# Wil-Lee/NN_BVH

Hardware: AMD Instinct MI355X
Metric: Mray/s (closest-hit + any-hit) (higher is better)
Workload: dtype f32; 1 GPU; crown, 1000x1400: one wavefront pass of 8 spp per step (8 spp per GPU-film) — primary, bounce-1 and bounce-2 closest-hit, shadow any-hit towards the light quads (batches pre-generated, hence independent: ONE launch; the dependent form is dependent_step), rays in --ray-order tile (a caller-side order the reference's integrator does not form: ray_order_probe), RecordShadowRayResult + RGBFilm::AddSam; sample_sets=4, geometry=procedural stand-in for crown (3548192 tris; data/crown.npz absent), tree=sah, triangles=3548192, nodes=7032259, rays_primary=11200000, rays_bounce=7410327, rays_bounce2=4392209, parallelism=tile-sharded x1, BVH replicated, film all-gather after the pass

## Files before the change

### nn_bvh_amd/csrc/bvh_trace.hip

```cpp
#include <hip/hip_runtime.h>
#include <stdint.h>

#include "bvh_trace.h"
#include "anim_math.h"
#include "spawn_math.h"
#include "stream_access.h"
#include "trace_math.h"

namespace nnbvh {

constexpr int kDone = (int)0x80000000;
constexpr int kReturn = (int)0x80000001;
constexpr int kEnter = (int)0x80000002;

#ifndef NNBVH_MINW_CLOSEST
#define NNBVH_MINW_CLOSEST 6
#endif
#ifndef NNBVH_MINW_ANY
#define NNBVH_MINW_ANY 6
#endif
#ifndef NNBVH_LEAN_EXTRA_WAVES
#define NNBVH_LEAN_EXTRA_WAVES 2
#endif
#ifndef NNBVH_MINW_ALPHA
#define NNBVH_MINW_ALPHA 5
#endif
#ifndef NNBVH_MINW_ALPHA_PATCH
#define NNBVH_MINW_ALPHA_PATCH 3
#endif
#ifndef NNBVH_ANIM_ENTER_WEIGHT
#define NNBVH_ANIM_ENTER_WEIGHT 8
#endif
template <typename T>
__device__ __forceinline__ T pick_batch(const T (&a)[kMaxFusedBatches], int b) {
    static_assert(kMaxFusedBatches == 4, "written out for four batches");
    return b == 0 ? a[0] : (b == 1 ? a[1] : (b == 2 ? a[2] : a[3]));
}

template <int MODE, int W, int INST, int PATCH, int ALPHA = 0, int SOA = 0, int HOSTC = 0>
__global__ __launch_bounds__(kBlockThreads, (INST ? 1 : (ALPHA ? (ALPHA == 2 ? NNBVH_MINW_ALPHA_PATCH : NNBVH_MINW_ALPHA) : ((MODE == 0 || MODE == 3) ? NNBVH_MINW_CLOSEST : NNBVH_MINW_ANY) + (PATCH ? 0 : NNBVH_LEAN_EXTRA_WAVES))))
void trace_kernel(TraceParams p) {
    static_assert(PATCH || !INST, "two-level scenes need the ray direction");
    static_assert(PATCH || !ALPHA, "the alpha test hashes the ray direction");
    static_assert(!HOSTC || (PATCH && (MODE == 0 || MODE == 2 || (MODE == 3 && !ALPHA && W == 8)) && !SOA),
                  "candidate mode: general instances of modes 0 / 2 / 3");
    __shared__ float s_stack[kBlockThreads / 64][W][2][64];
    constexpr bool kLean = !PATCH && !INST;
    constexpr int kColdRi = 0, kColdD = 1, kColdHit = kLean ? 0 : (PATCH ? 4 : 1),
                  kColdHost = kColdHit + ((MODE == 0 || MODE == 3) ? 4 : 0);
    constexpr int kColdBase = kColdHost + (kLean ? 0 : 1);
    constexpr int kSaveO = kColdBase, kSaveInv = kColdBase + 3, kSaveShear = kColdBase + 6,
                  kSaveKz = kColdBase + 9, kSaveTmax = kColdBase + 10, kSaveD = kColdBase + 11,
                  kResume = kColdBase + 14, kCurInst = kColdBase + 15, kHitInst = kColdBase + 16,
                  kInnerHit = kColdBase + 17, kColdTime = kColdBase + 18, kPendSlot = kColdBase + 19;
    constexpr int kColdFields = kColdBase + (INST ? 20 : 0);
    __shared__ float s_cold[kBlockThreads / 64][kColdFields > 0 ? kColdFields : 1][64];

    const int lane = threadIdx.x & 63;
    const int wave = threadIdx.x >> 6;
    const int gtid = blockIdx.x * kBlockThreads + threadIdx.x;
    float(*stk)[2][64] = s_stack[wave];
    float(*cold)[64] = s_cold[wave];
    int riReg = -1;
    if (!kLean) cold[kColdRi][lane] = __int_as_float(-1);
    const long spillStride = (long)gridDim.x * kBlockThreads;

    int q = 0;
    if (p.nQueues > 1) {
        unsigned xcc;
        asm volatile("s_getreg_b32 %0, hwreg(HW_REG_XCC_ID)" : "=s"(xcc));
        q = (int)(xcc & 0xf) % p.nQueues;
    }
    int queuesTried = 0;
    int curBatch = 0;
    long nRays = p.n;
    if (p.nDev) {
        const long nd = (long)*p.nDev;
        nRays = nd < 0 ? 0 : (nd < nRays ? nd : nRays);
    }

#ifdef NNBVH_STATS
    unsigned long long st[16] = {0, 0, 0, 0, 0, 0, 0, 0, 0, 0, 0, 0, 0, 0, 0, 0};
    unsigned long long stPrev = __builtin_amdgcn_s_memtime();
    int stKind = 2;
#endif
    RayState r;
    RayMasks masks = {0ull, 0ull, 0ull, 0ull, 0ull, 0ull};
    float tMax = 0.0f;
    int visited = 0, tests = 0;
    int cur = kDone, sp = 0, base = 0;
    int floor = -1;
    bool found = false;
    bool exhausted = false;

    auto pop_entry = [&](int &ref, float &key) {
        --sp;
        ref = __float_as_int(stk[sp & (W - 1)][0][lane]);
        key = stk[sp & (W - 1)][1][lane];
        asm volatile("" : "+v"(ref), "+v"(key));
        if (sp < base) {
            const uint2 e = p.spill[(long)sp * spillStride + gtid];
            base = sp;
            ref = (int)e.x;
            key = __uint_as_float(e.y);
            asm volatile("" : "+v"(ref), "+v"(key));
        }
        if (MODE != 2) visited += 1;
    };
    auto pop_next = [&]() -> int {
        const int lowest = (INST && floor > 0) ? floor : 0;
        const int none = (INST && floor >= 0) ? kReturn : kDone;
        if (sp <= lowest) return none;
        int ref;
        float key;
        pop_entry(ref, key);
        if (key < tMax) return ref;
        while (sp > lowest) {
            pop_entry(ref, key);
            if (key < tMax) return ref;
        }
        return none;
    };

    auto enter_instance = [&](int slot, unsigned flags, float4 s0, float4 s1, float4 s2) {
        const float4 s3 = p.prims[slot + 3], s4 = p.prims[slot + 4], s5 = p.prims[slot + 5];
        const V3 dOuter = {cold[kColdD][lane], cold[kColdD + 1][lane], cold[kColdD + 2][lane]};
        cold[kSaveO][lane] = r.o.x;
        cold[kSaveO + 1][lane] = r.o.y;
        cold[kSaveO + 2][lane] = r.o.z;
        cold[kSaveInv][lane] = r.inv.x;
        cold[kSaveInv + 1][lane] = r.inv.y;
        cold[kSaveInv + 2][lane] = r.inv.z;
        cold[kSaveShear][lane] = r.sx;
        cold[kSaveShear + 1][lane] = r.sy;
        cold[kSaveShear + 2][lane] = r.sz;
        cold[kSaveKz][lane] = __int_as_float(r.kz);
        cold[kSaveTmax][lane] = tMax;
        cold[kSaveD][lane] = dOuter.x;
        cold[kSaveD + 1][lane] = dOuter.y;
        cold[kSaveD + 2][lane] = dOuter.z;
        cold[kResume][lane] = __int_as_float((flags & kPrimLast) ? kDone : ~(slot + 6));
        cold[kCurInst][lane] = __int_as_float(__float_as_int(s0.w) + 1);
        cold[kInnerHit][lane] = 0.0f;
        V3 oIn, dIn;
        float4 m0 = s2, m1 = s3, m2 = s4;
        if (INST == 2 && (flags & kPrimAnimated) && p.anim)
            anim_inverse_rows(p.anim + (long)kAnimStride * __float_as_int(s0.w), cold[kColdTime][lane], m0, m1, m2);
        apply_inverse_ray(m0, m1, m2, r.o, dOuter, tMax, oIn, dIn);
        r.o = oIn;
        cold[kColdD][lane] = dIn.x;
        cold[kColdD + 1][lane] = dIn.y;
        cold[kColdD + 2][lane] = dIn.z;
        r.inv = {1.0f / dIn.x, 1.0f / dIn.y, 1.0f / dIn.z};
        ray_shear(r, dIn);
        floor = sp;
        if (MODE != 2) visited += 1;
        float tEntry;
        const bool rootHit =
            slab_partial(s0.x, s0.y, s0.z, s1.x, s1.y, s1.z, r, tEntry) && (tEntry < tMax);
        cur = rootHit ? __float_as_int(s5.x) : kReturn;
    };

    auto leave_instance = [&]() {
        const bool innerHit = cold[kInnerHit][lane] != 0.0f;
        r.o = {cold[kSaveO][lane], cold[kSaveO + 1][lane], cold[kSaveO + 2][lane]};
        r.inv = {cold[kSaveInv][lane], cold[kSaveInv + 1][lane], cold[kSaveInv + 2][lane]};
        r.sx = cold[kSaveShear][lane];
        r.sy = cold[kSaveShear + 1][lane];
        r.sz = cold[kSaveShear + 2][lane];
        r.kz = __float_as_int(cold[kSaveKz][lane]);
        cold[kColdD][lane] = cold[kSaveD][lane];
        cold[kColdD + 1][lane] = cold[kSaveD + 1][lane];
        cold[kColdD + 2][lane] = cold[kSaveD + 2][lane];
        if (!innerHit) tMax = cold[kSaveTmax][lane];
        cold[kCurInst][lane] = 0.0f;
        floor = -1;
        const int resume = __float_as_int(cold[kResume][lane]);
        cur = (resume == kDone) ? pop_next() : resume;
    };

    auto prim_math = [&](const int slot, const float4 s0, const float4 s1, const float4 s2) {
        const unsigned flags = __float_as_uint(s1.w);
        if (INST && (flags & kPrimInstance)) {
            if (INST == 2 && NNBVH_ANIM_ENTER_WEIGHT > 0 && (flags & kPrimAnimated) && p.anim) {
                cold[kPendSlot][lane] = __int_as_float(slot);
                cur = kEnter;
            } else {
                enter_instance(slot, flags, s0, s1, s2);
            }
        } else if (!kLean && (flags & kPrimHost)) {
            if constexpr (HOSTC) {
                const int c = __float_as_int(cold[kColdHost][lane]);
                if (c >= 0) {
                    long ray = __float_as_int(cold[kColdRi][lane]);
                    int cap = p.hcCap;
                    int32_t *hcPrim = p.hcPrim, *hcInst = p.hcInst;
                    if constexpr (MODE == 3) {
                        const int b = (int)(ray >> kFusedIndexBits);
                        ray &= (1 << kFusedIndexBits) - 1;
                        cap = pick_batch(p.bHcCap, b);
                        hcPrim = pick_batch(p.bHcPrim, b);
                        hcInst = pick_batch(p.bHcInst, b);
                    }
                    if (c < cap) {
                        const long at = ray * cap + c;
                        hcPrim[at] = __float_as_int(s0.w);
                        hcInst[at] = INST ? __float_as_int(cold[kCurInst][lane]) : 0;
                    }
                    cold[kColdHost][lane] = __int_as_float(c < cap ? c + 1 : -1);
                }
            } else {
                cold[kColdHost][lane] = 1.0f;
            }
            cur = (flags & kPrimLast) ? pop_next() : ~(slot + 3);
        } else {
            tests += 1;
            bool hit;
            float x0, x1, x2, th;
            int next;
            if (!PATCH || !(flags & kPrimPatch)) {
                hit = triangle_test(r, tMax, (flags & kPrimDegenerate) != 0,
                                    {s0.x, s0.y, s0.z}, {s1.x, s1.y, s1.z},
                                    {s2.x, s2.y, s2.z}, x0, x1, x2, th, kLean ? &masks : nullptr);
                next = slot + ((ALPHA && (flags & kPrimSmooth)) ? 6 : 3);
                if (ALPHA && hit && (flags & kPrimAlpha)) {
                    const float a = s2.w;
                    if (a < 1) {
                        const V3 rd = {cold[kColdD][lane], cold[kColdD + 1][lane],
                                       cold[kColdD + 2][lane]};
                        const float u = (a <= 0) ? 1.f : hash_float_6f(r.o, rd);
                        if (u > a) {
                            hit = false;
                            RayState rn = r;
                            if (flags & kPrimSmooth) {
                                const float4 m0 = p.prims[slot + 3], m1 = p.prims[slot + 4], m2 = p.prims[slot + 5];
                                rn.o = alpha_retrace_origin({s0.x, s0.y, s0.z}, {s1.x, s1.y, s1.z}, {s2.x, s2.y, s2.z}, x0,
                                                            x1, x2, (flags & kPrimFlipN) != 0, rd, true, {m0.x, m0.y, m0.z},
                                                            {m1.x, m1.y, m1.z}, {m2.x, m2.y, m2.z});
                            } else {
                                rn.o = alpha_retrace_origin({s0.x, s0.y, s0.z}, {s1.x, s1.y, s1.z},
                                                            {s2.x, s2.y, s2.z}, x0, x1, x2,
                                                            (flags & kPrimFlipN) != 0, rd);
                            }
                            tests += 1;
                            float y0, y1, y2, tn;
                            if (triangle_test(rn, tMax - th, (flags & kPrimDegenerate) != 0,
                                              {s0.x, s0.y, s0.z}, {s1.x, s1.y, s1.z},
                                              {s2.x, s2.y, s2.z}, y0, y1, y2, tn))
                                cold[kColdHost][lane] = HOSTC ? __int_as_float(-2) : 1.0f;
                        }
                    }
                }
            } else {
                const float4 s3 = p.prims[slot + 3];
                x2 = 0.0f;
                const V3 rd = {cold[PATCH ? kColdD : 0][lane], cold[PATCH ? kColdD + 1 : 0][lane],
                               cold[PATCH ? kColdD + 2 : 0][lane]};
                next = slot + 4 + ((ALPHA == 2 && (flags & kPrimSmooth)) ? 4 : 0) + ((ALPHA == 2 && (flags & kPrimUV)) ? 2 : 0);
                if constexpr (ALPHA == 2) {
                    constexpr int kAlphaPatchDepth = 3;
                    const float a = (flags & kPrimAlpha) ? s2.w : 1.0f;
                    RayState rn = r;
                    float tm = tMax, t0 = 0.0f, t1 = 0.0f, t2 = 0.0f;
                    int k = 0;
                    for (;;) {
                        hit = patch_test(rn, rd, tm, {s0.x, s0.y, s0.z}, {s1.x, s1.y, s1.z}, {s2.x, s2.y, s2.z},
                                         {s3.x, s3.y, s3.z}, x0, x1, th);
                        if (!hit || !(a < 1)) break;
                        const float u = (a <= 0) ? 1.f : hash_float_6f(rn.o, rd);
                        if (!(u > a)) break;
                        if (k == kAlphaPatchDepth) {
                            hit = false;
                            cold[kColdHost][lane] = HOSTC ? __int_as_float(-2) : 1.0f;
                            break;
                        }
                        if (k == 0) t0 = th;
                        else if (k == 1) t1 = th;
                        else t2 = th;
                        ++k;
                        rn.o = patch_retrace_origin({s0.x, s0.y, s0.z}, {s1.x, s1.y, s1.z}, {s2.x, s2.y, s2.z},
                                                    {s3.x, s3.y, s3.z}, x0, x1, (flags & kPrimFlipN) != 0, rd,
                                                    (flags & kPrimSmooth) != 0, (flags & kPrimUV) != 0,
                                                    p.prims + slot + 4);
                        tm = tm - th;
                        tests += 1;
                    }
                    if (hit && k > 0) {
                        if (k == 3) th = th + t2;
                        if (k >= 2) th = th + t1;
                        th = th + t0;
                    }
                } else {
                    hit = patch_test(r, rd, tMax, {s0.x, s0.y, s0.z}, {s1.x, s1.y, s1.z},
                                     {s2.x, s2.y, s2.z}, {s3.x, s3.y, s3.z}, x0, x1, th);
                }
            }
            bool closestLane = MODE == 0;
            if (MODE == 3 && hit)
                closestLane = !((p.anyMask >> ((kLean ? riReg : __float_as_int(cold[kColdRi][lane])) >> kFusedIndexBits)) & 1u);
            if (hit) {
                if (closestLane) {
                    cold[kColdHit][lane] = s0.w;
                    cold[kColdHit + 1][lane] = x0;
                    cold[kColdHit + 2][lane] = x1;
                    cold[kColdHit + 3][lane] = x2;
                    tMax = th;
                    if (INST) {
                        cold[kHitInst][lane] = cold[kCurInst][lane];
                        cold[kInnerHit][lane] = 1.0f;
                    }
                    if constexpr (HOSTC && MODE == 0) {
                        const int c = __float_as_int(cold[kColdHost][lane]);
                        if (c > 0) p.hcBefore[__float_as_int(cold[kColdRi][lane])] = c;
                    }
                    if constexpr (HOSTC && MODE == 3) {
                        const int c = __float_as_int(cold[kColdHost][lane]);
                        if (c > 0) {
                            const int tag = __float_as_int(cold[kColdRi][lane]);
                            pick_batch(p.bHcBefore, tag >> kFusedIndexBits)[tag & ((1 << kFusedIndexBits) - 1)] = c;
                        }
                    }
                } else {
                    found = true;
                }
            }
            if (MODE != 0 && found) cur = kDone;
            else if (flags & kPrimLast) cur = pop_next();
            else cur = ~next;
        }
    };

    auto interior_math = [&](const float4 q0, const float4 q1, const float4 q2, const float4 q3) {
        const int ref0 = __float_as_int(q3.x), ref1 = __float_as_int(q3.y);
        const int axis = __float_as_int(q3.z);
        const bool swap = ((r.kz >> axis) & 1) != 0;
        const float k0 = kLean ? slab_entry_key(q0.x, q0.y, q0.z, q0.w, q1.x, q1.y, r, masks)
                               : slab_entry_key(q0.x, q0.y, q0.z, q0.w, q1.x, q1.y, r);
        const float k1 = kLean ? slab_entry_key(q1.z, q1.w, q2.x, q2.y, q2.z, q2.w, r, masks)
                               : slab_entry_key(q1.z, q1.w, q2.x, q2.y, q2.z, q2.w, r);
        const int nearRef = swap ? ref1 : ref0, farRef = swap ? ref0 : ref1;
        const float nearT = swap ? k1 : k0, farT = swap ? k0 : k1;
        visited += 1;
        const bool doPush = (MODE == 1) || (farT < __builtin_inff());
        if (doPush && sp - base == W - 1) {
            uint2 e;
            e.x = __float_as_uint(stk[base & (W - 1)][0][lane]);
            e.y = __float_as_uint(stk[base & (W - 1)][1][lane]);
            p.spill[(long)base * spillStride + gtid] = e;
            ++base;
        }
        stk[sp & (W - 1)][0][lane] = __int_as_float(farRef);
        stk[sp & (W - 1)][1][lane] = farT;
        sp += doPush ? 1 : 0;
        if (MODE == 0 || MODE == 3) visited += doPush ? 0 : 1;
        cur = nearT < tMax ? nearRef : pop_next();
    };
    auto interior_step = [&]() {
#ifdef NNBVH_STATS
        st[14] += 1;
        st[15] += __popcll(__ballot(cur >= 0));
#endif
        if (cur >= 0) {
            const float4 *rec = kLean ? reinterpret_cast<const float4 *>(reinterpret_cast<const char *>(p.wide) + ((unsigned)cur << 6))
                                      : p.wide + 4 * (long)cur;
            const float4 q3 = rec[3];
            const float4 q0 = rec[0], q1 = rec[1], q2 = rec[2];
            interior_math(q0, q1, q2, q3);
        }
    };

    for (;;) {
#ifdef NNBVH_STATS
        {
            const unsigned long long now = __builtin_amdgcn_s_memtime();
            st[10 + stKind] += now - stPrev;
            stPrev = now;
        }
#endif
        const bool isInt = cur >= 0;
        const bool isIdle = cur == kDone;
        const int nInt = __popcll(__ballot(isInt));
        const unsigned long long idleMask = __ballot(isIdle);
        const int nIdle = __popcll(idleMask);
        const int nEnter = (INST == 2 && NNBVH_ANIM_ENTER_WEIGHT > 0) ? __popcll(__ballot(cur == kEnter)) : 0;
        const int nPrim = 64 - nInt - nIdle - nEnter;

        const int sI = nInt * 16, sP = nPrim * p.primWeight;
        const int sR = exhausted ? 0 : nIdle * p.refillWeight;
#ifdef NNBVH_STATS
        unsigned long long &stTrips = (nIdle == 64 || (sR > sI && sR > sP)) ? st[4]
                                      : ((sP > sI || nInt == 0) ? st[2] : st[0]);
        (&stTrips)[0] += 1;
        (&stTrips)[1] += (nIdle == 64 || (sR > sI && sR > sP)) ? nIdle
                         : ((sP > sI || nInt == 0) ? nPrim : nInt);
        stKind = (&stTrips == &st[4]) ? 2 : ((&stTrips == &st[2]) ? 1 : 0);
        if (&stTrips == &st[0]) {
            st[6] += nInt;
            st[7] += nPrim;
            st[8] += nIdle;
        }
#endif
        if (nIdle == 64 || (sR > sI && sR > sP)) {
            const int ri = isIdle ? (kLean ? riReg : __float_as_int(cold[kColdRi][lane])) : -1;
            if constexpr (MODE == 3 && HOSTC) {
                if (ri >= 0) {
                    const int b = ri >> kFusedIndexBits;
                    const long idx = ri & ((1 << kFusedIndexBits) - 1);
                    void *outp = pick_batch(p.bOut, b);
                    const int c = __float_as_int(cold[kColdHost][lane]);
                    if (pick_batch(p.bHcCap, b) > 0) pick_batch(p.bHcCount, b)[idx] = c;
                    if ((p.anyMask >> b) & 1u) {
                        store_stream(reinterpret_cast<uint8_t *>(outp) + idx, (uint8_t)(found ? 1 : (c != 0 ? 2 : 0)));
                    } else {
                        float4 h0, h1;
                        h0.x = cold[kColdHit][lane];
                        h0.y = tMax;
                        h0.z = cold[kColdHit + 1][lane];
                        h0.w = cold[kColdHit + 2][lane];
                        h1.x = cold[kColdHit + 3][lane];
                        h1.y = __int_as_float(visited);
                        h1.z = __int_as_float(tests);
                        h1.w = INST ? cold[kHitInst][lane] : 0.0f;
                        if (c < 0) h1.w = __int_as_float(-1);
                        float4 *out = reinterpret_cast<float4 *>(outp) + 2 * idx;
                        store_stream(out, h0);
                        store_stream(out + 1, h1);
                    }
                }
            } else if (MODE == 3 && ri >= 0) {
                const int b = ri >> kFusedIndexBits;
                const long idx = ri & ((1 << kFusedIndexBits) - 1);
                void *outp = b == 0 ? p.bOut[0] : (b == 1 ? p.bOut[1] : (b == 2 ? p.bOut[2] : p.bOut[3]));
                const bool needHost = !kLean && p.hasHostPrims && cold[kColdHost][lane] != 0.0f;
                if ((p.anyMask >> b) & 1u) {
                    store_stream(reinterpret_cast<uint8_t *>(outp) + idx, (uint8_t)(found ? 1 : (needHost ? 2 : 0)));
                } else {
                    float4 h0, h1;
                    h0.x = cold[kColdHit][lane];
                    h0.y = tMax;
                    h0.z = cold[kColdHit + 1][lane];
                    h0.w = cold[kColdHit + 2][lane];
                    h1.x = cold[kColdHit + 3][lane];
                    h1.y = __int_as_float(visited);
                    h1.z = __int_as_float(tests);
                    h1.w = INST ? cold[kHitInst][lane] : 0.0f;
                    if (needHost) h1.w = __int_as_float(-1);
                    float4 *out = reinterpret_cast<float4 *>(outp) + 2 * idx;
                    store_stream(out, h0);
                    store_stream(out + 1, h1);
                }
            } else if (ri >= 0) {
                if (MODE == 0) {
                    float4 h0, h1;
                    h0.x = cold[kColdHit][lane];
                    h0.y = tMax;
                    h0.z = cold[kColdHit + 1][lane];
                    h0.w = cold[kColdHit + 2][lane];
                    h1.x = cold[kColdHit + 3][lane];
                    h1.y = __int_as_float(visited);
                    h1.z = __int_as_float(tests);
                    h1.w = INST ? cold[kHitInst][lane] : 0.0f;
                    if constexpr (HOSTC) {
                        const int c = __float_as_int(cold[kColdHost][lane]);
                        if (c < 0) h1.w = __int_as_float(-1);
                        p.hcCount[ri] = c;
                    } else if (!kLean && p.hasHostPrims && cold[kColdHost][lane] != 0.0f) {
                        h1.w = __int_as_float(-1);
                    }
                    float4 *out = reinterpret_cast<float4 *>(p.hits) + 2 * (long)ri;
                    store_stream(out, h0);
                    store_stream(out + 1, h1);
                } else {
                    bool needHost;
                    if constexpr (HOSTC) {
                        const int c = __float_as_int(cold[kColdHost][lane]);
                        needHost = c != 0;
                        p.hcCount[ri] = c;
                    } else {
                        needHost = !kLean && p.hasHostPrims && cold[kColdHost][lane] != 0.0f;
                    }
                    store_stream(&p.occluded[ri], (uint8_t)(found ? 1 : (needHost ? 2 : 0)));
                    if (MODE == 1) {
                        if (p.visitedOut) store_stream(&p.visitedOut[ri], (int32_t)visited);
                        if (p.testsOut) store_stream(&p.testsOut[ri], (int32_t)tests);
                    }
                }
            }
            int newRi = -1;
            if (exhausted) break;
            long start = 0;
            for (;;) {
                if (MODE == 3) {
                    nRays = p.bN[curBatch];
                    if (const int32_t *nd = p.bNDev[curBatch]) {
                        const long v = *nd;
                        nRays = v < 0 ? 0 : (v < nRays ? v : nRays);
                    }
                }
                static_assert(kMaxQueues == 8, "queue ranges are computed with a shift by 3");
                const int qShift = p.nQueues > 1 ? 3 : 0;
                const long qBegin = (nRays * q) >> qShift, qEnd = (nRays * (q + 1)) >> qShift;
                unsigned got = 0;
                if (lane == 0)
                    got = atomicAdd(&p.queue[((MODE == 3 ? curBatch * p.nQueues : 0) + q) * kQueueStrideWords],
                                    (unsigned)nIdle);
                got = __builtin_amdgcn_readfirstlane(got);
                start = qBegin + (long)got;
                if (start < qEnd) {
                    const int rank = __builtin_amdgcn_mbcnt_hi(
                        (unsigned)(idleMask >> 32),
                        __builtin_amdgcn_mbcnt_lo((unsigned)idleMask, 0u));
                    if (isIdle && start + rank < qEnd) newRi = (int)(start + rank);
                    break;
                }
                if (++queuesTried >= p.nQueues) {
                    if (MODE == 3 && curBatch + 1 < p.nBatches) {
                        ++curBatch;
                        queuesTried = 0;
                        continue;
                    }
                    exhausted = true;
                    break;
                }
                q = (q + 1 == p.nQueues) ? 0 : q + 1;
            }
            if (isIdle) {
                const int tag = (MODE == 3 && newRi >= 0) ? (newRi | (curBatch << kFusedIndexBits)) : newRi;
                if (kLean) riReg = tag;
                else cold[kColdRi][lane] = __int_as_float(tag);
            }
            if (newRi >= 0) {
                const nnbvh_ray *batchRays = MODE == 3 ? p.bRays[curBatch] : p.rays;
                float4 r0, r1;
                if (!SOA || batchRays) {
                    const float4 *in = reinterpret_cast<const float4 *>(batchRays) + 2 * (long)newRi;
                    r0 = load_stream(in);
                    r1 = load_stream(in + 1);
                } else {
                    const nnbvh_ray_soa &q = MODE == 3 ? p.bSoa[curBatch] : p.soa;
                    auto ld = [&](const float *a) { return load_stream(a + newRi); };
                    r0 = {ld(q.ox), ld(q.oy), ld(q.oz), q.tmax ? ld(q.tmax) : __builtin_inff()};
                    r1 = {ld(q.dx), ld(q.dy), ld(q.dz), q.time ? ld(q.time) : 0.0f};
                }
                r.o = {r0.x, r0.y, r0.z};
                tMax = r0.w;
                const V3 d = {r1.x, r1.y, r1.z};
                if (PATCH) {
                    cold[kColdD][lane] = d.x;
                    cold[kColdD + 1][lane] = d.y;
                    cold[kColdD + 2][lane] = d.z;
                }
                r.inv = {1.0f / d.x, 1.0f / d.y, 1.0f / d.z};
                ray_shear(r, d);
                if (MODE == 0 || MODE == 3) {
                    cold[kColdHit][lane] = __int_as_float(-1);
                    cold[kColdHit + 1][lane] = 0.0f;
                    cold[kColdHit + 2][lane] = 0.0f;
                    cold[kColdHit + 3][lane] = 0.0f;
                }
                if (INST) {
                    cold[kHitInst][lane] = 0.0f;
                    cold[kCurInst][lane] = 0.0f;
                    cold[kColdTime][lane] = r1.w;
                    floor = -1;
                }
                if (!kLean && (HOSTC || p.hasHostPrims)) cold[kColdHost][lane] = 0.0f;
                visited = 1;
                tests = 0;
                found = false;
                sp = base = 0;
                float tEntry;
                const bool rootHit =
                    slab_partial(p.rootMin[0], p.rootMin[1], p.rootMin[2], p.rootMax[0],
                                 p.rootMax[1], p.rootMax[2], r, tEntry) &&
                    (tEntry < tMax);
                cur = rootHit ? p.rootRef : kDone;
            }
            if (kLean) masks = ray_masks(r);
            continue;
        }

        if (INST == 2 && NNBVH_ANIM_ENTER_WEIGHT > 0 && nEnter > 0 &&
            ((nInt == 0 && nPrim == 0) || (nEnter * NNBVH_ANIM_ENTER_WEIGHT > sI && nEnter * NNBVH_ANIM_ENTER_WEIGHT > sP))) {
            if (cur == kEnter) {
                const int slot = __float_as_int(cold[kPendSlot][lane]);
                const float4 s0 = p.prims[slot], s1 = p.prims[slot + 1], s2 = p.prims[slot + 2];
                enter_instance(slot, __float_as_uint(s1.w), s0, s1, s2);
            }
            continue;
        }

        if (sP > sI || nInt == 0) {
            const int nPrep = (MODE == 3) ? 1 : p.primRepeat;
            int prep = 0;
            do {
            if (cur < 0 && cur != kDone) {
                if (INST && cur == kReturn) leave_instance();
                if (cur < 0 && cur != kDone && cur != kReturn && (INST != 2 || cur != kEnter)) {
                    const int slot = ~cur;
                    const float4 *pr = kLean ? reinterpret_cast<const float4 *>(reinterpret_cast<const char *>(p.prims) + ((unsigned)slot << 4))
                                             : p.prims + slot;
                    float4 s0 = pr[0], s1 = pr[1], s2 = pr[2];
                    asm volatile("" : "+v"(s0.x), "+v"(s0.y), "+v"(s0.z), "+v"(s0.w), "+v"(s1.x), "+v"(s1.y),
                                      "+v"(s1.z), "+v"(s1.w), "+v"(s2.x), "+v"(s2.y), "+v"(s2.z), "+v"(s2.w));
                    prim_math(slot, s0, s1, s2);
                }
            }
            } while (++prep < nPrep && __ballot(cur < 0 && cur != kDone) != 0ull);
        } else {
            if (MODE == 3) {
                interior_step();
                if (p.intRepeat > 1 && __ballot(cur >= 0) != 0ull) {
                    interior_step();
                    if (p.intRepeat > 2 && __ballot(cur >= 0) != 0ull) {
                        interior_step();
                        for (int rep = 3; rep < p.intRepeat && __ballot(cur >= 0) != 0ull; ++rep) interior_step();
                    }
                }
            } else {
            int rep = 0;
            do {
                interior_step();
            } while (++rep < p.intRepeat && __ballot(cur >= 0) != 0ull);
            }
        }
    }
#ifdef NNBVH_STATS
    if (lane == 0 && p.stats)
        for (int k = 0; k < 16; ++k) atomicAdd(&p.stats[k], st[k]);
#endif
}

template <int MODE, int W, int INST, int PATCH, int ALPHA = 0, int SOA = 0, int HOSTC = 0>
static hipError_t launch_one(const TraceParams &p, int blocks, hipStream_t stream, int *occupancy) {
    if (occupancy) {
        return hipOccupancyMaxActiveBlocksPerMultiprocessor(
            occupancy, trace_kernel<MODE, W, INST, PATCH, ALPHA, SOA, HOSTC>, kBlockThreads, 0);
    }
    hipLaunchKernelGGL((trace_kernel<MODE, W, INST, PATCH, ALPHA, SOA, HOSTC>), dim3((unsigned)blocks),
                       dim3(kBlockThreads), 0, stream, p);
    return hipGetLastError();
}

template <int MODE, int ALPHA, int HOSTC>
static hipError_t launch_inst(const TraceParams &p, int instanced, int blocks, hipStream_t stream, int *occupancy) {
    if (!instanced) return launch_one<MODE, 8, 0, 1, ALPHA, 0, HOSTC>(p, blocks, stream, occupancy);
    return p.anim ? launch_one<MODE, 8, 2, 1, ALPHA, 0, HOSTC>(p, blocks, stream, occupancy)
                  : launch_one<MODE, 8, 1, 1, ALPHA, 0, HOSTC>(p, blocks, stream, occupancy);
}
template <int MODE, int HOSTC>
static hipError_t launch_general(const TraceParams &p, int instanced, int patches, int blocks, hipStream_t stream,
                                 int *occupancy) {
    if (patches & 4) return launch_inst<MODE, 2, HOSTC>(p, instanced, blocks, stream, occupancy);
    if (patches & 2) return launch_inst<MODE, 1, HOSTC>(p, instanced, blocks, stream, occupancy);
    return launch_inst<MODE, 0, HOSTC>(p, instanced, blocks, stream, occupancy);
}

static hipError_t launch_fused(const TraceParams &p, int window, int instanced, int patches, int blocks,
                               hipStream_t stream, int *occupancy) {
    if (window != 8 || (patches & 2)) return hipErrorInvalidValue;
    if (p.hcCap > 0) {
        if (instanced) return p.anim ? launch_one<3, 8, 2, 1, 0, 0, 1>(p, blocks, stream, occupancy)
                                     : launch_one<3, 8, 1, 1, 0, 0, 1>(p, blocks, stream, occupancy);
        return launch_one<3, 8, 0, 1, 0, 0, 1>(p, blocks, stream, occupancy);
    }
    if (instanced) return p.anim ? launch_one<3, 8, 2, 1>(p, blocks, stream, occupancy)
                                 : launch_one<3, 8, 1, 1>(p, blocks, stream, occupancy);
    bool soa = false;
    for (int b = 0; b < p.nBatches; ++b) soa = soa || !p.bRays[b];
    if (!patches && !p.hasHostPrims && p.fits32)
        return soa ? launch_one<3, 8, 0, 0, 0, 1>(p, blocks, stream, occupancy) : launch_one<3, 8, 0, 0>(p, blocks, stream, occupancy);
    if (soa) return hipErrorInvalidValue;
    return launch_one<3, 8, 0, 1>(p, blocks, stream, occupancy);
}

template <int MODE>
static hipError_t launch_mode(const TraceParams &p, int window, int instanced, int patches, int blocks,
                              hipStream_t stream, int *occupancy) {
    if constexpr (MODE == 0 || MODE == 2) {
        if (p.hcCap > 0) return launch_general<MODE, 1>(p, instanced, patches, blocks, stream, occupancy);
    }
    if (instanced || (patches & 6)) return launch_general<MODE, 0>(p, instanced, patches, blocks, stream, occupancy);
    const bool soa = !p.rays && !occupancy;
    if (!patches && !p.hasHostPrims && p.fits32 && window == 8 && !instanced) {
        if (soa && MODE != 1) return launch_one<MODE == 1 ? 0 : MODE, 8, 0, 0, 0, 1>(p, blocks, stream, occupancy);
        if (!soa) return launch_one<MODE, 8, 0, 0>(p, blocks, stream, occupancy);
    }
    if (soa) return hipErrorInvalidValue;
    switch (window) {
    case 4: return launch_one<MODE, 4, 0, 1>(p, blocks, stream, occupancy);
    case 8: return launch_one<MODE, 8, 0, 1>(p, blocks, stream, occupancy);
    case 16: return launch_one<MODE, 16, 0, 1>(p, blocks, stream, occupancy);
    default: return hipErrorInvalidValue;
    }
}

__global__ void zero_queue_kernel(unsigned *queue, int words) {
    for (int i = threadIdx.x; i < words; i += blockDim.x) queue[i] = 0u;
}
hipError_t launch_zero_queue(unsigned *queue, int words, hipStream_t stream) {
    hipLaunchKernelGGL(zero_queue_kernel, dim3(1), dim3(256), 0, stream, queue, words);
    return hipGetLastError();
}

__global__ void zero_words_kernel(int32_t *words, long n) {
    for (long i = (long)blockIdx.x * blockDim.x + threadIdx.x; i < n; i += (long)gridDim.x * blockDim.x) words[i] = 0;
}
hipError_t launch_zero_words(int32_t *words, long n, int maxBlocks, hipStream_t stream) {
    long blocks = (n + 255) / 256;
    blocks = blocks < 1 ? 1 : (blocks < maxBlocks ? blocks : maxBlocks);
    hipLaunchKernelGGL(zero_words_kernel, dim3((unsigned)blocks), dim3(256), 0, stream, words, n);
    return hipGetLastError();
}

hipError_t launch_trace(int mode, const TraceParams &p, int window, int instanced, int patches, int blocks,
                        hipStream_t stream, int *occupancy) {
    switch (mode) {
    case 0: return launch_mode<0>(p, window, instanced, patches, blocks, stream, occupancy);
    case 1: return launch_mode<1>(p, window, instanced, patches, blocks, stream, occupancy);
    case 2: return launch_mode<2>(p, window, instanced, patches, blocks, stream, occupancy);
    case 3: return launch_fused(p, window, instanced, patches, blocks, stream, occupancy);
    default: return hipErrorInvalidValue;
    }
}

}
```

### nn_bvh_amd/csrc/trace_math.h

```cpp
#pragma once
#include <hip/hip_runtime.h>
#include <stdint.h>

namespace nnbvh {

#define DEV static __device__ __forceinline__

DEV constexpr float gamma_f(int n) {
    return ((float)n * 0x1p-24f) / (1.0f - (float)n * 0x1p-24f);
}

DEV float dop(float a, float b, float c, float d) {
    float cd = c * d;
    float diff = __builtin_fmaf(a, b, -cd);
    float err = __builtin_fmaf(-c, d, cd);
    return diff + err;
}

DEV float fmax3(float a, float b, float c) {
    return __builtin_fmaxf(__builtin_fmaxf(a, b), c);
}
DEV float max3(float a, float b, float c) {
    float m = a;
    if (m < b) m = b;
    if (m < c) m = c;
    return m;
}

struct V3 {
    float x, y, z;
};
DEV V3 cross(V3 v, V3 w) {
    return {dop(v.y, w.z, v.z, w.y), dop(v.z, w.x, v.x, w.z), dop(v.x, w.y, v.y, w.x)};
}
DEV float dot(V3 v, V3 w) { return v.x * w.x + v.y * w.y + v.z * w.z; }
DEV float len2(V3 v) { return v.x * v.x + v.y * v.y + v.z * v.z; }
DEV V3 sub(V3 a, V3 b) { return {a.x - b.x, a.y - b.y, a.z - b.z}; }
DEV float maxabs(V3 v) { return max3(__builtin_fabsf(v.x), __builtin_fabsf(v.y), __builtin_fabsf(v.z)); }
DEV float sel3(V3 v, int k) { return k == 0 ? v.x : (k == 1 ? v.y : v.z); }

struct RayState {
    V3 o, inv;
    float sx, sy, sz;
    int kz;
};

DEV void ray_shear(RayState &r, V3 d) {
    float ax = __builtin_fabsf(d.x), ay = __builtin_fabsf(d.y), az = __builtin_fabsf(d.z);
    int kz = (ax > ay) ? ((ax > az) ? 0 : 2) : ((ay > az) ? 1 : 2);
    int kx = kz + 1;
    if (kx == 3) kx = 0;
    int ky = kx + 1;
    if (ky == 3) ky = 0;
    float dx = kx == 0 ? d.x : (kx == 1 ? d.y : d.z);
    float dy = ky == 0 ? d.x : (ky == 1 ? d.y : d.z);
    float dz = kz == 0 ? d.x : (kz == 1 ? d.y : d.z);
    r.sx = -dx / dz;
    r.sy = -dy / dz;
    r.sz = 1.0f / dz;
    r.kz = (kz << 8) | (r.inv.x < 0.0f ? 1 : 0) | (r.inv.y < 0.0f ? 2 : 0) | (r.inv.z < 0.0f ? 4 : 0);
}

struct RayMasks {
    unsigned long long negX, negY, negZ;
    unsigned long long k0, k1, k2;
};
DEV RayMasks ray_masks(const RayState &r) {
    const int kz = r.kz >> 8;
    return {__ballot(r.inv.x < 0.0f), __ballot(r.inv.y < 0.0f), __ballot(r.inv.z < 0.0f),
            __ballot(kz == 0), __ballot(kz == 1), __ballot(kz == 2)};
}
DEV float sel_m(unsigned long long m, float a, float b) {
    float out;
    asm("v_cndmask_b32_e64 %0, %2, %1, %3" : "=v"(out) : "v"(a), "v"(b), "s"(m));
    return out;
}

DEV bool slab_partial(float mnx, float mny, float mnz, float mxx, float mxy, float mxz,
                      const RayState &r, float &tEntry) {
    constexpr float widen = 1.0f + 2.0f * gamma_f(3);
    float tMin = (((r.inv.x < 0.0f) ? mxx : mnx) - r.o.x) * r.inv.x;
    float tMax = (((r.inv.x < 0.0f) ? mnx : mxx) - r.o.x) * r.inv.x;
    float tyMin = (((r.inv.y < 0.0f) ? mxy : mny) - r.o.y) * r.inv.y;
    float tyMax = (((r.inv.y < 0.0f) ? mny : mxy) - r.o.y) * r.inv.y;
    tMax *= widen;
    tyMax *= widen;
    const bool out1 = (tMin > tyMax) | (tyMin > tMax);
    tMin = (tyMin > tMin) ? tyMin : tMin;
    tMax = (tyMax < tMax) ? tyMax : tMax;
    float tzMin = (((r.inv.z < 0.0f) ? mxz : mnz) - r.o.z) * r.inv.z;
    float tzMax = (((r.inv.z < 0.0f) ? mnz : mxz) - r.o.z) * r.inv.z;
    tzMax *= widen;
    const bool out2 = (tMin > tzMax) | (tzMin > tMax);
    tMin = (tzMin > tMin) ? tzMin : tMin;
    tMax = (tzMax < tMax) ? tzMax : tMax;
    tEntry = tMin;
    return !(out1 | out2) & (tMax > 0.0f);
}

DEV float slab_entry_key(float mnx, float mny, float mnz, float mxx, float mxy, float mxz, const RayState &r) {
    constexpr float widen = 1.0f + 2.0f * gamma_f(3);
    const float ax = (((r.inv.x < 0.0f) ? mxx : mnx) - r.o.x) * r.inv.x;
    const float bx = (((r.inv.x < 0.0f) ? mnx : mxx) - r.o.x) * r.inv.x;
    const float ay = (((r.inv.y < 0.0f) ? mxy : mny) - r.o.y) * r.inv.y;
    const float by = (((r.inv.y < 0.0f) ? mny : mxy) - r.o.y) * r.inv.y;
    const float az = (((r.inv.z < 0.0f) ? mxz : mnz) - r.o.z) * r.inv.z;
    const float bz = (((r.inv.z < 0.0f) ? mnz : mxz) - r.o.z) * r.inv.z;
    const float a = __builtin_fmaxf(__builtin_fmaxf(ax, ay), az);
    const float b = __builtin_fminf(__builtin_fminf(bx, by), bz) * widen;
    const bool ok = !__builtin_isunordered(ax, bx) & (a <= b) & (b > 0.0f);
    return ok ? a : __builtin_inff();
}

DEV float slab_entry_key(float mnx, float mny, float mnz, float mxx, float mxy, float mxz, const RayState &r,
                         const RayMasks &m) {
    constexpr float widen = 1.0f + 2.0f * gamma_f(3);
    const float ax = (sel_m(m.negX, mxx, mnx) - r.o.x) * r.inv.x;
    const float bx = (sel_m(m.negX, mnx, mxx) - r.o.x) * r.inv.x;
    const float ay = (sel_m(m.negY, mxy, mny) - r.o.y) * r.inv.y;
    const float by = (sel_m(m.negY, mny, mxy) - r.o.y) * r.inv.y;
    const float az = (sel_m(m.negZ, mxz, mnz) - r.o.z) * r.inv.z;
    const float bz = (sel_m(m.negZ, mnz, mxz) - r.o.z) * r.inv.z;
    const float a = __builtin_fmaxf(__builtin_fmaxf(ax, ay), az);
    const float b = __builtin_fminf(__builtin_fminf(bx, by), bz) * widen;
    const bool ok = !__builtin_isunordered(ax, bx) & (a <= b) & (b > 0.0f);
    return ok ? a : __builtin_inff();
}

DEV bool triangle_test(const RayState &r, float tMax, bool degenerate, V3 p0, V3 p1, V3 p2,
                       float &b0, float &b1, float &b2, float &tHit, const RayMasks *m = nullptr) {
    if (degenerate) return false;
    V3 a = sub(p0, r.o), b = sub(p1, r.o), c = sub(p2, r.o);
    float p0x, p0y, p0z, p1x, p1y, p1z, p2x, p2y, p2z;
    if (m) {
        auto px = [&](V3 v) { return sel_m(m->k2, v.x, sel_m(m->k0, v.y, v.z)); };
        auto py = [&](V3 v) { return sel_m(m->k1, v.x, sel_m(m->k2, v.y, v.z)); };
        auto pz = [&](V3 v) { return sel_m(m->k0, v.x, sel_m(m->k1, v.y, v.z)); };
        p0x = px(a), p0y = py(a), p0z = pz(a);
        p1x = px(b), p1y = py(b), p1z = pz(b);
        p2x = px(c), p2y = py(c), p2z = pz(c);
    } else {
        const int kz = r.kz >> 8;
        int kx = kz + 1;
        if (kx == 3) kx = 0;
        int ky = kx + 1;
        if (ky == 3) ky = 0;
        p0x = sel3(a, kx), p0y = sel3(a, ky), p0z = sel3(a, kz);
        p1x = sel3(b, kx), p1y = sel3(b, ky), p1z = sel3(b, kz);
        p2x = sel3(c, kx), p2y = sel3(c, ky), p2z = sel3(c, kz);
    }
    const float sx = r.sx, sy = r.sy, sz = r.sz;
    p0x += sx * p0z;
    p0y += sy * p0z;
    p1x += sx * p1z;
    p1y += sy * p1z;
    p2x += sx * p2z;
    p2y += sy * p2z;
    float e0 = dop(p1x, p2y, p1y, p2x);
    float e1 = dop(p2x, p0y, p2y, p0x);
    float e2 = dop(p0x, p1y, p0y, p1x);
    if (e0 == 0.0f || e1 == 0.0f || e2 == 0.0f) {
        double p2txp1ty = (double)p2x * (double)p1y;
        double p2typ1tx = (double)p2y * (double)p1x;
        e0 = (float)(p2typ1tx - p2txp1ty);
        double p0txp2ty = (double)p0x * (double)p2y;
        double p0typ2tx = (double)p0y * (double)p2x;
        e1 = (float)(p0typ2tx - p0txp2ty);
        double p1txp0ty = (double)p1x * (double)p0y;
        double p1typ0tx = (double)p1y * (double)p0x;
        e2 = (float)(p1typ0tx - p1txp0ty);
    }
    if ((e0 < 0 || e1 < 0 || e2 < 0) && (e0 > 0 || e1 > 0 || e2 > 0)) return false;
    float det = e0 + e1 + e2;
    if (det == 0) return false;
    p0z *= sz;
    p1z *= sz;
    p2z *= sz;
    float tScaled = e0 * p0z + e1 * p1z + e2 * p2z;
    if (det < 0 && (tScaled >= 0 || tScaled < tMax * det)) return false;
    else if (det > 0 && (tScaled <= 0 || tScaled > tMax * det)) return false;
    float invDet = 1.0f / det;
    float t = tScaled * invDet;
    const bool firstIsNan = __builtin_isunordered(p0z, p0x) | __builtin_isunordered(p0y, e0);
    float maxZt = fmax3(__builtin_fabsf(p0z), __builtin_fabsf(p1z), __builtin_fabsf(p2z));
    float deltaZ = gamma_f(3) * maxZt;
    float maxXt = fmax3(__builtin_fabsf(p0x), __builtin_fabsf(p1x), __builtin_fabsf(p2x));
    float maxYt = fmax3(__builtin_fabsf(p0y), __builtin_fabsf(p1y), __builtin_fabsf(p2y));
    float deltaX = gamma_f(5) * (maxXt + maxZt);
    float deltaY = gamma_f(5) * (maxYt + maxZt);
    float deltaE = 2.0f * (gamma_f(2) * maxXt * maxYt + deltaY * maxXt + deltaX * maxYt);
    float maxE = fmax3(__builtin_fabsf(e0), __builtin_fabsf(e1), __builtin_fabsf(e2));
    float deltaT = 3.0f * (gamma_f(3) * maxE * maxZt + deltaE * maxZt + deltaZ * maxE) *
                   __builtin_fabsf(invDet);
    if (!firstIsNan & (t <= deltaT)) return false;
    b0 = e0 * invDet;
    b1 = e1 * invDet;
    b2 = e2 * invDet;
    tHit = t;
    return true;
}

DEV bool quadratic(float a, float b, float c, float &t0, float &t1) {
    if (a == 0) {
        if (b == 0) return false;
        t0 = t1 = -c / b;
        return true;
    }
    float discrim = dop(b, b, 4.0f * a, c);
    if (discrim < 0) return false;
    float root = __builtin_sqrtf(discrim);
    float q = -0.5f * (b + __builtin_copysignf(root, b));
    t0 = q / a;
    t1 = c / q;
    if (t0 > t1) {
        float s = t0;
        t0 = t1;
        t1 = s;
    }
    return true;
}

DEV float det3(V3 r0, V3 r1, V3 r2) {
    float minor12 = dop(r1.y, r2.z, r1.z, r2.y);
    float minor02 = dop(r1.x, r2.z, r1.z, r2.x);
    float minor01 = dop(r1.x, r2.y, r1.y, r2.x);
    return __builtin_fmaf(r0.z, minor01, dop(r0.x, minor12, r0.y, minor02));
}

DEV V3 lerp3(float t, V3 a, V3 b) {
    float omt = 1.0f - t;
    return {omt * a.x + t * b.x, omt * a.y + t * b.y, omt * a.z + t * b.z};
}

DEV void patch_root(float u, const RayState &r, V3 rd, V3 p00, V3 p10, V3 p01, V3 p11, float &vnum,
                    float &tnum, float &p2) {
    V3 uo = lerp3(u, p00, p10);
    V3 ud = sub(lerp3(u, p01, p11), uo);
    V3 deltao = sub(uo, r.o);
    V3 perp = cross(rd, ud);
    p2 = len2(perp);
    vnum = det3({deltao.x, rd.x, perp.x}, {deltao.y, rd.y, perp.y}, {deltao.z, rd.z, perp.z});
    tnum = det3({deltao.x, ud.x, perp.x}, {deltao.y, ud.y, perp.y}, {deltao.z, ud.z, perp.z});
}

DEV bool patch_test(const RayState &r, V3 rd, float tMax, V3 p00, V3 p10, V3 p01, V3 p11, float &uOut,
                    float &vOut, float &tOut) {
    float a = dot(cross(sub(p10, p00), sub(p01, p11)), rd);
    float c = dot(cross(sub(p00, r.o), rd), sub(p01, p00));
    float b = dot(cross(sub(p10, r.o), rd), sub(p11, p10)) - (a + c);
    float u1, u2;
    if (!quadratic(a, b, c, u1, u2)) return false;
    float eps = gamma_f(10) * (maxabs(r.o) + maxabs(rd) + maxabs(p00) + maxabs(p10) +
                               maxabs(p01) + maxabs(p11));
    float t = tMax, u = 0.0f, v = 0.0f;
    if (0 <= u1 && u1 <= 1) {
        float v1, t1, p2;
        patch_root(u1, r, rd, p00, p10, p01, p11, v1, t1, p2);
        if (t1 > p2 * eps && 0 <= v1 && v1 <= p2) {
            u = u1;
            v = v1 / p2;
            t = t1 / p2;
        }
    }
    if (0 <= u2 && u2 <= 1 && u2 != u1) {
        float v2, t2, p2;
        patch_root(u2, r, rd, p00, p10, p01, p11, v2, t2, p2);
        t2 /= p2;
        if (0 <= v2 && v2 <= p2 && t > t2 && t2 > eps) {
            t = t2;
            u = u2;
            v = v2 / p2;
        }
    }
    if (t >= tMax) return false;
    uOut = u;
    vOut = v;
    tOut = t;
    return true;
}

DEV float next_up(float v) {
    if (__builtin_isinf(v) && v > 0.f) return v;
    if (v == -0.f) v = 0.f;
    unsigned ui = __float_as_uint(v);
    if (v >= 0) ++ui;
    else --ui;
    return __uint_as_float(ui);
}
DEV float next_down(float v) {
// ... 56 lines not shown
```

Baseline: 4787 Mray/s.

## Trim register pressure in lean fused closest-hit kernel via kernarg reloads and two-mask selects

```diff
diff --git a/nn_bvh_amd/csrc/bvh_trace.hip b/nn_bvh_amd/csrc/bvh_trace.hip
--- a/nn_bvh_amd/csrc/bvh_trace.hip
+++ b/nn_bvh_amd/csrc/bvh_trace.hip
@@ -30,6 +30,9 @@
 #endif
 #ifndef NNBVH_ANIM_ENTER_WEIGHT
 #define NNBVH_ANIM_ENTER_WEIGHT 8
+#endif
+#ifndef NNBVH_FUSED_PRIM_LOOP
+#define NNBVH_FUSED_PRIM_LOOP 1
 #endif
 template <typename T>
 __device__ __forceinline__ T pick_batch(const T (&a)[kMaxFusedBatches], int b) {
@@ -46,6 +49,7 @@
                   "candidate mode: general instances of modes 0 / 2 / 3");
     __shared__ float s_stack[kBlockThreads / 64][W][2][64];
     constexpr bool kLean = !PATCH && !INST;
+    constexpr bool kDiet = kLean && MODE == 3;
     constexpr int kColdRi = 0, kColdD = 1, kColdHit = kLean ? 0 : (PATCH ? 4 : 1),
                   kColdHost = kColdHit + ((MODE == 0 || MODE == 3) ? 4 : 0);
     constexpr int kColdBase = kColdHost + (kLean ? 0 : 1);
@@ -64,6 +68,24 @@
     int riReg = -1;
     if (!kLean) cold[kColdRi][lane] = __int_as_float(-1);
     const long spillStride = (long)gridDim.x * kBlockThreads;
+    auto args = [&]() -> const TraceParams & {
+        if constexpr (kDiet) {
+            auto *k = (const __attribute__((address_space(4))) char *)__builtin_amdgcn_kernarg_segment_ptr();
+            asm volatile("" : "+s"(k));
+            return *(const TraceParams *)k;
+        } else {
+            return p;
+        }
+    };
+    auto spill_slot = [&](int level) -> uint2 * {
+        if constexpr (kDiet) {
+            unsigned blocks = gridDim.x;
+            asm volatile("" : "+s"(blocks));
+            return args().spill + ((long)level * ((long)blocks * kBlockThreads) + gtid);
+        } else {
+            return p.spill + ((long)level * spillStride + gtid);
+        }
+    };
 
     int q = 0;
     if (p.nQueues > 1) {
@@ -85,7 +107,7 @@
     int stKind = 2;
 #endif
     RayState r;
-    RayMasks masks = {0ull, 0ull, 0ull, 0ull, 0ull, 0ull};
+    RayMasks masks = {0ull, 0ull, 0ull, 0ull, 0ull};
     float tMax = 0.0f;
     int visited = 0, tests = 0;
     int cur = kDone, sp = 0, base = 0;
@@ -99,7 +121,7 @@
         key = stk[sp & (W - 1)][1][lane];
         asm volatile("" : "+v"(ref), "+v"(key));
         if (sp < base) {
-            const uint2 e = p.spill[(long)sp * spillStride + gtid];
+            const uint2 e = *spill_slot(sp);
             base = sp;
             ref = (int)e.x;
             key = __uint_as_float(e.y);
@@ -346,7 +368,7 @@
             uint2 e;
             e.x = __float_as_uint(stk[base & (W - 1)][0][lane]);
             e.y = __float_as_uint(stk[base & (W - 1)][1][lane]);
-            p.spill[(long)base * spillStride + gtid] = e;
+            *spill_slot(base) = e;
             ++base;
         }
         stk[sp & (W - 1)][0][lane] = __int_as_float(farRef);
@@ -401,15 +423,25 @@
         }
 #endif
         if (nIdle == 64 || (sR > sI && sR > sP)) {
+            const TraceParams &a = args();
+            struct {
+                int nQueues, nBatches, rootRef;
+                unsigned *queue;
+                float mn[3], mx[3];
+            } ra = {a.nQueues, a.nBatches, a.rootRef, a.queue, {a.rootMin[0], a.rootMin[1], a.rootMin[2]},
+                    {a.rootMax[0], a.rootMax[1], a.rootMax[2]}};
+            if constexpr (kDiet)
+                asm volatile("" : "+s"(ra.nQueues), "+s"(ra.nBatches), "+s"(ra.rootRef), "+s"(ra.queue), "+s"(ra.mn[0]),
+                                  "+s"(ra.mn[1]), "+s"(ra.mn[2]), "+s"(ra.mx[0]), "+s"(ra.mx[1]), "+s"(ra.mx[2]));
             const int ri = isIdle ? (kLean ? riReg : __float_as_int(cold[kColdRi][lane])) : -1;
             if constexpr (MODE == 3 && HOSTC) {
                 if (ri >= 0) {
                     const int b = ri >> kFusedIndexBits;
                     const long idx = ri & ((1 << kFusedIndexBits) - 1);
-                    void *outp = pick_batch(p.bOut, b);
+                    void *outp = pick_batch(a.bOut, b);
                     const int c = __float_as_int(cold[kColdHost][lane]);
-                    if (pick_batch(p.bHcCap, b) > 0) pick_batch(p.bHcCount, b)[idx] = c;
-                    if ((p.anyMask >> b) & 1u) {
+                    if (pick_batch(a.bHcCap, b) > 0) pick_batch(a.bHcCount, b)[idx] = c;
+                    if ((a.anyMask >> b) & 1u) {
                         store_stream(reinterpret_cast<uint8_t *>(outp) + idx, (uint8_t)(found ? 1 : (c != 0 ? 2 : 0)));
                     } else {
                         float4 h0, h1;
@@ -430,9 +462,9 @@
             } else if (MODE == 3 && ri >= 0) {
                 const int b = ri >> kFusedIndexBits;
                 const long idx = ri & ((1 << kFusedIndexBits) - 1);
-                void *outp = b == 0 ? p.bOut[0] : (b == 1 ? p.bOut[1] : (b == 2 ? p.bOut[2] : p.bOut[3]));
-                const bool needHost = !kLean && p.hasHostPrims && cold[kColdHost][lane] != 0.0f;
-                if ((p.anyMask >> b) & 1u) {
+                void *outp = b == 0 ? a.bOut[0] : (b == 1 ? a.bOut[1] : (b == 2 ? a.bOut[2] : a.bOut[3]));
+                const bool needHost = !kLean && a.hasHostPrims && cold[kColdHost][lane] != 0.0f;
+                if ((a.anyMask >> b) & 1u) {
                     store_stream(reinterpret_cast<uint8_t *>(outp) + idx, (uint8_t)(found ? 1 : (needHost ? 2 : 0)));
                 } else {
                     float4 h0, h1;
@@ -463,11 +495,11 @@
                     if constexpr (HOSTC) {
                         const int c = __float_as_int(cold[kColdHost][lane]);
                         if (c < 0) h1.w = __int_as_float(-1);
-                        p.hcCount[ri] = c;
-                    } else if (!kLean && p.hasHostPrims && cold[kColdHost][lane] != 0.0f) {
+                        a.hcCount[ri] = c;
+                    } else if (!kLean && a.hasHostPrims && cold[kColdHost][lane] != 0.0f) {
                         h1.w = __int_as_float(-1);
                     }
-                    float4 *out = reinterpret_cast<float4 *>(p.hits) + 2 * (long)ri;
+                    float4 *out = reinterpret_cast<float4 *>(a.hits) + 2 * (long)ri;
                     store_stream(out, h0);
                     store_stream(out + 1, h1);
                 } else {
@@ -475,14 +507,14 @@
                     if constexpr (HOSTC) {
                         const int c = __float_as_int(cold[kColdHost][lane]);
                         needHost = c != 0;
-                        p.hcCount[ri] = c;
+                        a.hcCount[ri] = c;
                     } else {
-                        needHost = !kLean && p.hasHostPrims && cold[kColdHost][lane] != 0.0f;
-                    }
-                    store_stream(&p.occluded[ri], (uint8_t)(found ? 1 : (needHost ? 2 : 0)));
+                        needHost = !kLean && a.hasHostPrims && cold[kColdHost][lane] != 0.0f;
+                    }
+                    store_stream(&a.occluded[ri], (uint8_t)(found ? 1 : (needHost ? 2 : 0)));
                     if (MODE == 1) {
-                        if (p.visitedOut) store_stream(&p.visitedOut[ri], (int32_t)visited);
-                        if (p.testsOut) store_stream(&p.testsOut[ri], (int32_t)tests);
+                        if (a.visitedOut) store_stream(&a.visitedOut[ri], (int32_t)visited);
+                        if (a.testsOut) store_stream(&a.testsOut[ri], (int32_t)tests);
                     }
                 }
             }
@@ -491,18 +523,18 @@
             long start = 0;
             for (;;) {
                 if (MODE == 3) {
-                    nRays = p.bN[curBatch];
-                    if (const int32_t *nd = p.bNDev[curBatch]) {
+                    nRays = a.bN[curBatch];
+                    if (const int32_t *nd = a.bNDev[curBatch]) {
                         const long v = *nd;
                         nRays = v < 0 ? 0 : (v < nRays ? v : nRays);
                     }
                 }
                 static_assert(kMaxQueues == 8, "queue ranges are computed with a shift by 3");
-                const int qShift = p.nQueues > 1 ? 3 : 0;
+                const int qShift = ra.nQueues > 1 ? 3 : 0;
                 const long qBegin = (nRays * q) >> qShift, qEnd = (nRays * (q + 1)) >> qShift;
                 unsigned got = 0;
                 if (lane == 0)
-                    got = atomicAdd(&p.queue[((MODE == 3 ? curBatch * p.nQueues : 0) + q) * kQueueStrideWords],
+                    got = atomicAdd(&ra.queue[((MODE == 3 ? curBatch * ra.nQueues : 0) + q) * kQueueStrideWords],
                                     (unsigned)nIdle);
                 got = __builtin_amdgcn_readfirstlane(got);
                 start = qBegin + (long)got;
@@ -513,8 +545,8 @@
                     if (isIdle && start + rank < qEnd) newRi = (int)(start + rank);
                     break;
                 }
-                if (++queuesTried >= p.nQueues) {
-                    if (MODE == 3 && curBatch + 1 < p.nBatches) {
+                if (++queuesTried >= ra.nQueues) {
+                    if (MODE == 3 && curBatch + 1 < ra.nBatches) {
                         ++curBatch;
                         queuesTried = 0;
                         continue;
@@ -522,7 +554,7 @@
                     exhausted = true;
                     break;
                 }
-                q = (q + 1 == p.nQueues) ? 0 : q + 1;
+                q = (q + 1 == ra.nQueues) ? 0 : q + 1;
             }
             if (isIdle) {
                 const int tag = (MODE == 3 && newRi >= 0) ? (newRi | (curBatch << kFusedIndexBits)) : newRi;
@@ -530,14 +562,14 @@
                 else cold[kColdRi][lane] = __int_as_float(tag);
             }
             if (newRi >= 0) {
-                const nnbvh_ray *batchRays = MODE == 3 ? p.bRays[curBatch] : p.rays;
+                const nnbvh_ray *batchRays = MODE == 3 ? a.bRays[curBatch] : a.rays;
                 float4 r0, r1;
                 if (!SOA || batchRays) {
                     const float4 *in = reinterpret_cast<const float4 *>(batchRays) + 2 * (long)newRi;
                     r0 = load_stream(in);
                     r1 = load_stream(in + 1);
                 } else {
-                    const nnbvh_ray_soa &q = MODE == 3 ? p.bSoa[curBatch] : p.soa;
+                    const nnbvh_ray_soa &q = MODE == 3 ? a.bSoa[curBatch] : a.soa;
                     auto ld = [&](const float *a) { return load_stream(a + newRi); };
                     r0 = {ld(q.ox), ld(q.oy), ld(q.oz), q.tmax ? ld(q.tmax) : __builtin_inff()};
                     r1 = {ld(q.dx), ld(q.dy), ld(q.dz), q.time ? ld(q.time) : 0.0f};
@@ -564,17 +596,17 @@
                     cold[kColdTime][lane] = r1.w;
                     floor = -1;
                 }
-                if (!kLean && (HOSTC || p.hasHostPrims)) cold[kColdHost][lane] = 0.0f;
+                if (!kLean && (HOSTC || a.hasHostPrims)) cold[kColdHost][lane] = 0.0f;
                 visited = 1;
                 tests = 0;
                 found = false;
                 sp = base = 0;
                 float tEntry;
                 const bool rootHit =
-                    slab_partial(p.rootMin[0], p.rootMin[1], p.rootMin[2], p.rootMax[0],
-                                 p.rootMax[1], p.rootMax[2], r, tEntry) &&
+                    slab_partial(ra.mn[0], ra.mn[1], ra.mn[2], ra.mx[0],
+                                 ra.mx[1], ra.mx[2], r, tEntry) &&
                     (tEntry < tMax);
-                cur = rootHit ? p.rootRef : kDone;
+                cur = rootHit ? ra.rootRef : kDone;
             }
             if (kLean) masks = ray_masks(r);
             continue;
@@ -591,7 +623,7 @@
         }
 
         if (sP > sI || nInt == 0) {
-            const int nPrep = (MODE == 3) ? 1 : p.primRepeat;
+            const int nPrep = (MODE == 3 && !(kDiet && NNBVH_FUSED_PRIM_LOOP)) ? 1 : p.primRepeat;
             int prep = 0;
             do {
             if (cur < 0 && cur != kDone) {
diff --git a/nn_bvh_amd/csrc/trace_math.h b/nn_bvh_amd/csrc/trace_math.h
--- a/nn_bvh_amd/csrc/trace_math.h
+++ b/nn_bvh_amd/csrc/trace_math.h
@@ -63,12 +63,12 @@
 
 struct RayMasks {
     unsigned long long negX, negY, negZ;
-    unsigned long long k0, k1, k2;
+    unsigned long long k0, k1;
 };
 DEV RayMasks ray_masks(const RayState &r) {
     const int kz = r.kz >> 8;
     return {__ballot(r.inv.x < 0.0f), __ballot(r.inv.y < 0.0f), __ballot(r.inv.z < 0.0f),
-            __ballot(kz == 0), __ballot(kz == 1), __ballot(kz == 2)};
+            __ballot(kz == 0), __ballot(kz == 1)};
 }
 DEV float sel_m(unsigned long long m, float a, float b) {
     float out;
@@ -133,8 +133,8 @@
     V3 a = sub(p0, r.o), b = sub(p1, r.o), c = sub(p2, r.o);
     float p0x, p0y, p0z, p1x, p1y, p1z, p2x, p2y, p2z;
     if (m) {
-        auto px = [&](V3 v) { return sel_m(m->k2, v.x, sel_m(m->k0, v.y, v.z)); };
-        auto py = [&](V3 v) { return sel_m(m->k1, v.x, sel_m(m->k2, v.y, v.z)); };
+        auto px = [&](V3 v) { return sel_m(m->k0, v.y, sel_m(m->k1, v.z, v.x)); };
+        auto py = [&](V3 v) { return sel_m(m->k1, v.x, sel_m(m->k0, v.z, v.y)); };
         auto pz = [&](V3 v) { return sel_m(m->k0, v.x, sel_m(m->k1, v.y, v.z)); };
         p0x = px(a), p0y = py(a), p0z = pz(a);
         p1x = px(b), p1y = py(b), p1z = pz(b);
diff --git a/nn_bvh_amd/kernel_figures.py b/nn_bvh_amd/kernel_figures.py
--- /dev/null
+++ b/nn_bvh_amd/kernel_figures.py
@@ -0,0 +1,110 @@
+import struct
+
+BUNDLE_MAGIC = b"__CLANG_OFFLOAD_BUNDLE__"
+NT_AMDGPU_METADATA = 32
+FIELDS = ("vgpr_count", "sgpr_count", "vgpr_spill_count", "sgpr_spill_count", "private_segment_fixed_size",
+          "group_segment_fixed_size")
+
+
+def _unpack(b, i):
+    t = b[i]
+    i += 1
+    if t <= 0x7f:
+        return t, i
+    if t >= 0xe0:
+        return t - 0x100, i
+    if 0xa0 <= t <= 0xbf:
+        n = t & 0x1f
+        return b[i:i + n].decode("utf-8", "replace"), i + n
+    if 0x90 <= t <= 0x9f or t in (0xdc, 0xdd):
+        n, i = (t & 0x0f, i) if t <= 0x9f else _uint(b, i, 2 if t == 0xdc else 4)
+        out = []
+        for _ in range(n):
+            v, i = _unpack(b, i)
+            out.append(v)
+        return out, i
+    if 0x80 <= t <= 0x8f or t in (0xde, 0xdf):
+        n, i = (t & 0x0f, i) if t <= 0x8f else _uint(b, i, 2 if t == 0xde else 4)
+        out = {}
+        for _ in range(n):
+            k, i = _unpack(b, i)
+            v, i = _unpack(b, i)
+            out[k] = v
+        return out, i
+    if t == 0xc0:
+        return None, i
+    if t in (0xc2, 0xc3):
+        return t == 0xc3, i
+    if t in (0xc4, 0xc5, 0xc6, 0xd9, 0xda, 0xdb):
+        n, i = _uint(b, i, {0xc4: 1, 0xc5: 2, 0xc6: 4, 0xd9: 1, 0xda: 2, 0xdb: 4}[t])
+        raw = b[i:i + n]
+        return (raw if t <= 0xc6 else raw.decode("utf-8", "replace")), i + n
+    if 0xcc <= t <= 0xcf:
+        return _uint(b, i, 1 << (t - 0xcc))
+    if 0xd0 <= t <= 0xd3:
+        n = 1 << (t - 0xd0)
+        return int.from_bytes(b[i:i + n], "big", signed=True), i + n
+    if t == 0xca:
+        return struct.unpack(">f", b[i:i + 4])[0], i + 4
+    if t == 0xcb:
+        return struct.unpack(">d", b[i:i + 8])[0], i + 8
+    raise ValueError(f"msgpack type 0x{t:02x} is not expected in code-object metadata")
+
+
+def _uint(b, i, n):
+    return int.from_bytes(b[i:i + n], "big"), i + n
+
+
+def code_object_metadata(elf):
+    if elf[:4] != b"\x7fELF" or elf[4] != 2:
+        return None
+    shoff, = struct.unpack_from("<Q", elf, 0x28)
+    shentsize, shnum = struct.unpack_from("<HH", elf, 0x3a)
+    for k in range(shnum):
+        sh = shoff + k * shentsize
+        sh_type, = struct.unpack_from("<I", elf, sh + 4)
+        off, size = struct.unpack_from("<QQ", elf, sh + 0x18)
+        if sh_type != 7:
+            continue
+        i, end = off, off + size
+        while i + 12 <= end:
+            namesz, descsz, ntype = struct.unpack_from("<III", elf, i)
+            name = elf[i + 12:i + 12 + namesz]
+            desc = i + 12 + ((namesz + 3) & ~3)
+            if ntype == NT_AMDGPU_METADATA and name.rstrip(b"\0") == b"AMDGPU":
+                return _unpack(elf[desc:desc + descsz], 0)[0]
+            i = desc + ((descsz + 3) & ~3)
+    return None
+
+
+def code_objects(blob, arch="gfx950"):
+    at = blob.find(BUNDLE_MAGIC)
+    if at < 0:
+        yield blob
+        return
+    while at >= 0:
+        n, = struct.unpack_from("<Q", blob, at + len(BUNDLE_MAGIC))
+        i = at + len(BUNDLE_MAGIC) + 8
+        for _ in range(n):
+            off, size, tlen = struct.unpack_from("<QQQ", blob, i)
+            triple = blob[i + 24:i + 24 + tlen].decode()
+            i += 24 + tlen
+            if size and triple.startswith("hip") and arch in triple:
+                yield blob[at + off:at + off + size]
+        at = blob.find(BUNDLE_MAGIC, at + len(BUNDLE_MAGIC))
+
+
+def kernel_figures(path, arch="gfx950"):
+    with open(path, "rb") as f:
+        blob = f.read()
+    out = {}
+    for elf in code_objects(blob, arch):
+        meta = code_object_metadata(elf)
+        for k in (meta or {}).get("amdhsa.kernels", []):
+            out[k[".name"]] = {key.lstrip("."): v for key, v in k.items() if key != ".args"}
+    return out
+
+
+def waves_per_simd(vgprs, max_waves=8, file_size=512, granule=8):
+    alloc = max(granule, (vgprs + granule - 1) // granule * granule)
+    return min(max_waves, file_size // alloc)
```

Measured after the change: 4809 Mray/s, median of 6. No clear change (+0.5%).
